# mackelab/poisson-gpfa

Hardware: AMD Instinct MI355X
Metric: EM iterations/sec (higher is better)
Workload: dtype f64

## Files before the change

### poisson-gpfa_amd/csrc/core.hip

```cpp
#include "ctx.h"
#include "model.h"
#include "dual.h"

using namespace pgpfa;

thread_local std::string g_err;
thread_local unsigned long long g_fail_count = 0;

int fail(const char* fmt, ...) {
  char buf[1024];
  va_list ap;
  va_start(ap, fmt);
  vsnprintf(buf, sizeof(buf), fmt, ap);
  va_end(ap);
  g_err = buf;
  ++g_fail_count;
  return 1;
}

int ensure_hbuf(pgpfa_ctx* c, size_t len) {
  if (len <= c->hbuf_len) return 0;
  if (c->hbuf) hipHostFree(c->hbuf);
  c->hbuf = nullptr;
  HIPC(hipHostMalloc((void**)&c->hbuf, len * sizeof(double)));
// ... 792 lines not shown
  rc |= dmalloc(c, &c->dual_tbl, (size_t)round_up(q, 128) * c->dual_ncol + 4096, true);
  rc |= dmalloc(c, &c->ppart, (size_t)p * (PACC_SPLITS + 1) * T * T + 256);
  c->vsmgp_ok.assign(R, 0);
  c->trial_snap.assign(R, -1);
  c->trial_dual.assign(R, 0);
  c->lam_resident.assign(R, 0);
  c->lam_valid.assign(R, 0);
  rc |= dmalloc(c, &c->Flr, slab * p + 256 * (size_t)c->Tp, true);
  rc |= dmalloc(c, &c->d_rank, p); rc |= dmalloc(c, &c->d_roff, p + 1); rc |= dmalloc(c, &c->d_roff16, p + 1);
  rc |= dmalloc(c, &c->d_cmap, (size_t)p * c->Tp + 2 * NB + 64); rc |= dmalloc(c, &c->d_nrtab, (size_t)p * c->Tp / 16 + 64);
  c->tab_cap = 4 * ((size_t)c->ld / 64 + 2 * (size_t)p + 4);
  rc |= dmalloc(c, &c->d_kr_ft, c->tab_cap); rc |= dmalloc(c, &c->d_kr_f, c->tab_cap);
  rc |= dmalloc(c, &c->sink, 128, true);
  rc |= dmalloc(c, &c->zero16, 2, true);
  rc |= dmalloc(c, &c->d_thin_ft, c->tab_cap); rc |= dmalloc(c, &c->d_thin_f, c->tab_cap); rc |= dmalloc(c, &c->d_thin_s, c->tab_cap);
  rc |= dmalloc(c, &c->Fbig, (size_t)c->ld * c->ld + 256 * (size_t)c->ld, true); rc |= dmalloc(c, &c->FTbig, (size_t)c->ld * c->ld + 256 * (size_t)c->ld, true);
  rc |= dmalloc(c, &c->Gbar, (size_t)T * p * p + 64); rc |= dmalloc(c, &c->Wtbar, (size_t)T * p * p + 64); rc |= dmalloc(c, &c->d_blk_lat, (size_t)p * c->Tp / 16 + 64); rc |= dmalloc(c, &c->d_blk_col, (size_t)p * c->Tp / 16 + 64);
  rc |= dmalloc(c, &c->vec, (size_t)q * (p + 1));
  rc |= dmalloc(c, &c->cdpart, (size_t)1024 * (p + 2) * q);
  rc |= dmalloc(c, &c->cdout, (size_t)(p + 2) * q + 8);
  rc |= dmalloc(c, &c->cdym, (size_t)(p + 1) * q + 8);
  rc |= dmalloc(c, &c->cdym_part, (size_t)1024 * (p + 1) * q);
  rc |= dmalloc(c, &c->last_trials, R);
  {
    const size_t NH = 1 + (size_t)(p + 1) + (size_t)(p + 1) * (p + 2) / 2;
    rc |= dmalloc(c, &c->cdhpart, (size_t)128 * NH * q);
    rc |= dmalloc(c, &c->cdhout, NH * q + 8);
    rc |= dmalloc(c, &c->cdcenter, (size_t)q * (p + 1));
    rc |= dmalloc(c, &c->cdpack, (size_t)q * (p + 3) + 8);
  }
  if (hipHostMalloc((void**)&c->h_pcg, 4 * sizeof(int), hipHostMallocMapped) != hipSuccess ||
      hipHostGetDevicePointer((void**)&c->d_hpcg, c->h_pcg, 0) != hipSuccess) { (void)hipGetLastError(); c->h_pcg = nullptr; c->d_hpcg = nullptr; }
  rc |= alloc_cholws(c, &c->kws, p * TAU_MULTI_MAX, c->Tp, true);
  c->kws.nact = round_up(T, 64);
  {
    const size_t nqmax = (size_t)p * TAU_MULTI_MAX;
    rc |= dmalloc(c, &c->tK, slab * nqmax); rc |= dmalloc(c, &c->tM, slab * nqmax); rc |= dmalloc(c, &c->tA1, slab * nqmax);
    rc |= dmalloc(c, &c->tA2, slab * nqmax);
    rc |= dmalloc(c, &c->tscal, 16 + 8 * nqmax); rc |= dmalloc(c, &c->tpart, 1024 + 64 * nqmax);
  }
  if (rc) { pgpfa_destroy(c); return 1; }
  e = hipStreamSynchronize(c->st);
  if (e != hipSuccess) { pgpfa_destroy(c); return fail("sync: %s", hipGetErrorString(e)); }
  if (const char* g = std::getenv("PGPFA_RANK_GRAN")) { const int v = std::atoi(g); if (v == 4 || v == 8 || v == 16) c->rank_gran = v; }
  c->info["n_pad"] = c->npad;
  c->info["counts_two_bytes"] = 0.0;
  c->info["trial_lengths_set"] = 0.0;
  c->info["observed_set"] = 0.0;
  c->info["last_cd_unobserved_neurons"] = 0.0;
  c->info["arena_bytes"] = 0.0;
  c->info["last_eps_wt_norm"] = 0.0;
  c->info["last_eps_wt_rms"] = 0.0;
  c->info["last_split_cov"] = 0.0;
  c->info["last_yt_mix_fused"] = 0.0;
  c->info["last_cov_f32"] = 0.0;
  c->info["last_cov_f32_fallbacks"] = 0.0;
  for (const char* k : {"plan_ms_total", "plans", "set_params_calls", "last_retry_ms", "last_dense_retries", "last_param_step", "last_param_step_prev",
                        "last_fallback_no_descent", "last_fallback_line_search", "last_fallback_outer_cap", "arena_grow_ms_total", "last_cold_restarts"}) c->info[k] = 0.0;
  *out = c;
  return 0;
}

int pgpfa_destroy(pgpfa_ctx* c) {
  if (!c) return 0;
  hipSetDevice(c->device);
  if (c->st) hipStreamSynchronize(c->st);
  if (c->comm) ncclCommDestroy(c->comm);
  for (void* p : c->allocs) hipFree(p);
  if (c->vsmgp) hipFree(c->vsmgp);
  if (c->Flr32) hipFree(c->Flr32);
  if (c->lam_keep) hipFree(c->lam_keep);
  if (c->split_buf) hipFree(c->split_buf);
  if (c->Yhi) hipFree(c->Yhi);
  if (c->trial_len) hipFree(c->trial_len);
  if (c->obs) hipFree(c->obs);
  arena_release(c);
  if (c->hbuf) hipHostFree(c->hbuf);
  if (c->dl_stage) hipHostFree(c->dl_stage);
  if (c->hibuf) hipHostFree(c->hibuf);
  if (c->ring) hipHostFree(c->ring);
  if (c->h_pcg) hipHostFree(c->h_pcg);
  if (c->h_seq) hipHostFree(c->h_seq);
  for (auto e : c->prof.pool) hipEventDestroy(e);
  if (c->st2) { hipStreamSynchronize(c->st2); hipStreamDestroy(c->st2); }
  if (c->tau_pin) hipHostFree(c->tau_pin);
  if (c->ev_tau_fork) hipEventDestroy(c->ev_tau_fork);
  if (c->ev_tau_done) hipEventDestroy(c->ev_tau_done);
  if (c->ev_fork) hipEventDestroy(c->ev_fork);
  if (c->ev_join) hipEventDestroy(c->ev_join);
  if (c->st) hipStreamDestroy(c->st);
  delete c;
  return 0;
}

int pgpfa_set_option(pgpfa_ctx* c, const char* key, double v) {
  if (!c || !key) return fail("null argument");
  const std::string k(key);
  if (k == "newton_xtol") c->xtol = v;
  else if (k == "newton_max_iter") c->max_iter = (int)v;
  else if (k == "use_mfma") {
    const bool was = c->mfma;
    c->mfma = (v != 0.0);
    if (c->have_params && c->rank_gran != 16 && was != c->mfma)
      CHK(pgpfa_set_params(c, std::vector<double>(c->hC).data(), std::vector<double>(c->hd).data(), std::vector<double>(c->htau).data()));
  }
  else if (k == "cd_mfma") c->cd_mfma = (v != 0.0);
  else if (k == "cd_hess_mfma") c->cd_hess_mfma = (v != 0.0);
  else if (k == "cross_kernel") c->cross_kernel = (v != 0.0);
  else if (k == "cd_debug") c->cd_debug = (int)v;
  else if (k == "pcg_fused") c->pcg_fused = (int)v;
  else if (k == "pcg_w32") c->pcg_w32 = (v != 0.0);
  else if (k == "pcg_form") c->pcg_form = (int)v;
  else if (k == "pcg_vec32") c->pcg_vec32 = (int)v;
  else if (k == "pcg_rx32") c->pcg_rx32 = (int)v;
  else if (k == "pcg_adapt") c->pcg_adapt = (int)v;
  else if (k == "pcg_xcd") c->pcg_xcd = (int)v;
  else if (k == "mt_fill") c->mt_fill = (int)v;
  else if (k == "overlap_factors") c->overlap_factors = (int)v;
  else if (k == "mix_slot") c->mix_slot = (int)v;
  else if (k == "yt_mix") c->yt_mix = (v != 0.0);
  else if (k == "pivchol_pairs") c->pivchol_pairs = (v != 0.0);
  else if (k == "vsm_b4") c->vsm_b4 = (int)v;
  else if (k == "poisson_tiles") c->poisson_tiles = (int)v;
  else if (k == "yt_mix_dbg") c->yt_mix_dbg = (int)v;
  else if (k == "yt_mix_dma") c->yt_mix_dma = (v != 0.0);
  else if (k == "syrk_dbg") c->syrk_dbg = (int)v;
  else if (k == "syrk_tile") c->syrk_tile = (int)v;
  else if (k == "mix_wide") c->mix_wide = (int)v;
  else if (k == "thin_products") {
    const bool was = c->thin_products >= 2;
    c->thin_products = (int)v;
    if (c->have_params && c->rank_gran != 16 && was != (c->thin_products >= 2))
      CHK(pgpfa_set_params(c, std::vector<double>(c->hC).data(), std::vector<double>(c->hd).data(), std::vector<double>(c->htau).data()));
  }
  else if (k == "copy_kernels") c->copy_kernels = (v != 0.0);
  else if (k == "chord") c->chord = (v != 0.0);
  else if (k == "shared_pcg") c->shared_pcg = (v != 0.0);
  else if (k == "time_newton") c->time_newton = (v != 0.0);
  else if (k == "pcg_trace") c->pcg_trace = (v != 0.0);
  else if (k == "measure_mix") { c->measure_mix = (v != 0.0); c->info["last_eps_wt_norm"] = 0.0; c->info["last_eps_wt_rms"] = 0.0; }
  else if (k == "pcg_retire") c->pcg_retire = (v != 0.0);
  else if (k == "split_cov") c->split_cov = (v != 0.0);
  else if (k == "split_max_norm") c->split_max_norm = v;
  else if (k == "cov_mode") c->cov_mode = (int)v;
  else if (k == "lowrank_tol") {
    const bool changed = c->lr_tol != v;
    c->lr_tol = v;
    if (c->have_params && changed)
      CHK(pgpfa_set_params(c, std::vector<double>(c->hC).data(), std::vector<double>(c->hd).data(), std::vector<double>(c->htau).data()));
  }
  else if (k == "keep_trial_vsmgp") c->keep_trial_vsmgp = (v != 0.0);
  else if (k == "dual_lowrank") c->dual_lowrank = (v != 0.0);
  else if (k == "dual_f32") c->dual_f32 = (int)v;
  else if (k == "laplace_f32") { if (v != 0.0 && v != 1.0 && v != 2.0) return fail("laplace_f32 is 0, 1 or 2"); c->laplace_f32 = (int)v; }
  else if (k == "laplace_evidence") { if (v != 0.0 && v != 1.0) return fail("laplace_evidence is 0 or 1"); c->laplace_evidence = (int)v; }
  else if (k == "sample_chunk_trials") { if (v < 0.0 || v != std::floor(v)) return fail("sample_chunk_trials is a count of trials, or 0"); c->sample_chunk = (int)v; }
  else if (k == "rates_chunk_trials") { if (v < 0.0 || v != std::floor(v)) return fail("rates_chunk_trials is a count of trials, or 0"); c->rates_chunk = (int)v; }
  else if (k == "slab_row_align") c->slab_row_align = (v != 0.0);
  else if (k == "vsm_mfma") c->vsm_mfma = (v != 0.0);
  else if (k == "dual_gemm") c->dual_gemm = (v != 0.0);
  else if (k == "extrapolate_start") c->extrapolate = (v != 0.0);
  else if (k == "extrapolate_beta") c->extrapolate_beta = v;
  else if (k == "extrapolate_guard") c->extrapolate_guard = v;
  else if (k == "start_guard") c->start_guard = (v != 0.0);
  else if (k == "shared_min") c->shared_min = (int)v;
  else if (k == "pcg_inner") c->pcg_inner_max = std::max(1, (int)v);
  else if (k == "pcg_eta0") c->pcg_eta0 = v;
  else if (k == "splitk_target") c->splitk_target = std::max(1, (int)v);
  else if (k == "small_tile_below") c->small_tile_below = (int)v;
  else if (k == "f32_tile64") c->f32_tile64 = (int)v;
  else if (k == "splitk_below64") c->splitk_below64 = (int)v;
  else if (k == "pcg_outer_max") c->pcg_outer_max = (int)v;
  else if (k == "chord_xtol") c->chord_xtol = v;
  else if (k == "chord_rho") c->chord_rho = v;
  else if (k == "chord_max_step") c->chord_max_step = v;
  else if (k == "chord_max") c->chord_max = (int)v;
  else if (k == "chunk_trials") { if (c->B > 0) return fail("chunk_trials must be set before the first E-step"); c->chunk_opt = (int)v; }
  else if (k == "workspace_headroom") c->arena_headroom = std::max(1.0, v);
  else if (k == "rank_gran") { if (v != 4.0 && v != 8.0 && v != 16.0) return fail("rank_gran is 4, 8 or 16"); c->rank_gran = (int)v; if (c->have_params) CHK(pgpfa_set_params(c, std::vector<double>(c->hC).data(), std::vector<double>(c->hd).data(), std::vector<double>(c->htau).data())); }
  else if (k == "workspace_pool") { if (c->arena_cap > 0) return fail("workspace_pool must be set before the first E-step"); c->use_pool = (v != 0.0); }
// ... 481 lines not shown
```

### poisson-gpfa_amd/csrc/cov.hip

```cpp
#include "ctx.h"
#include "model.h"
#include "split.h"
#include "ytmix.h"

using namespace pgpfa;

template <typename TIN>
void launch_post_vsm(pgpfa_ctx* c, const TIN* Mt, long long sM, int ncol, int ns, int full_range, const int* roff = nullptr, int ts = 0) {
  const int T = c->T, p = c->p;
  if (ts <= 0) ts = T;
  if (p > 10 && c->vsm_mfma) {
    const int CB = post_vsm_mfma_cb(p, sizeof(TIN) == 4);
    if (p <= 20 && c->vsm_b4) {
      constexpr int VW = 16 / (int)sizeof(TIN);
      const bool vec = c->vsm_b4 >= 2 && T % VW == 0 && ts % VW == 0 && c->ld % VW == 0 && sM % VW == 0 && (((size_t)Mt) & 15) == 0;
      auto go = [&](auto nbk, auto vv) {
        constexpr int NBK = decltype(nbk)::value;
        constexpr bool VEC = decltype(vv)::value;
        const size_t lds4 = (size_t)CB * post_vsm_b4_cs(p, VEC) * sizeof(TIN);
        constexpr int BINS = VEC ? 64 : 32;
        (void)hipFuncSetAttribute(reinterpret_cast<const void*>(&post_vsm_b4_kernel<NBK, TIN, VEC>), hipFuncAttributeMaxDynamicSharedMemorySize, (int)lds4);
        hipLaunchKernelGGL((post_vsm_b4_kernel<NBK, TIN, VEC>), dim3((T + BINS - 1) / BINS, ns), dim3(512), lds4, c->st, Mt, sM, c->ld, ncol, T, p, c->vsm,
                           c->ident, c->trial_of_slot, full_range, CB, roff, (int)GBN, ts);
      };
// ... 136 lines not shown
        a.ncmap = c->rank_compact ? round_up(c->rtot16, (int)NB) : 0;
        if (ytmix_lds(PW) + (size_t)a.ncmap * sizeof(int) > (size_t)160 * 1024) a.ncmap = 0;
        const size_t lds = ytmix_lds(PW) + (size_t)a.ncmap * sizeof(int);
        a.zero16 = c->zero16;
        const bool dma = c->yt_mix_dma && c->zero16 && (!a.cmap || a.ncmap > 0) && rpad % 2 == 0 && lw.sM % 2 == 0 && (reinterpret_cast<uintptr_t>(lw.Mt) & 15) == 0;
        auto launch = [&](auto kern) {
          (void)hipFuncSetAttribute(reinterpret_cast<const void*>(kern), hipFuncAttributeMaxDynamicSharedMemorySize, (int)lds);
          hipLaunchKernelGGL(kern, dim3((unsigned)(a.nbx * nb)), dim3(YTM_THREADS), lds, c->st, a);
        };
        if (dma) launch(&yt_mix_kernel<PW, true>); else launch(&yt_mix_kernel<PW, false>);
      }
    });
    prof_end(c);
  } else {
  prof_begin(c, TAG_MIX, (double)nb * T * (mix_cols * 8.0 + (double)p * ract * 4.0));
  if (p > 16)
    hipLaunchKernelGGL((mix_vsm_wide2_kernel<20, true>), dim3((T + 63) / 64, nb), dim3(256), 0, c->st, lw.H, (long long)lw.sH, c->ld, c->Gbin, sW, T, p, ract, c->eps,
                       c->vsm, c->ident, c->trial_of_slot, Ts, c->sink, D, sD, ldd);
  else
  dispatch_pw(p, [&](auto pw) {
    constexpr int PW = decltype(pw)::value;
    if constexpr (PW <= 10) {
      if (c->mix_slot >= 3 && p == PW && ract % 4 == 0) {
        (void)hipFuncSetAttribute(reinterpret_cast<const void*>(&mix_slot3_kernel<PW, 128, 2>), hipFuncAttributeMaxDynamicSharedMemorySize, (int)mix_slot_lds(PW, 128));
        hipLaunchKernelGGL((mix_slot3_kernel<PW, 128, 2>), dim3((T + 127) / 128, nb), dim3(256), mix_slot_lds(PW, 128), c->st, (const double*)lw.H, (long long)lw.sH, c->ld, D, sD, ldd,
                           c->Gbin, sW, T, ract, c->eps, c->vsm, c->ident, c->trial_of_slot, c->d_roff, ctile, Ts);
        return;
      }
      if (c->mix_slot >= 2 && p == PW && ract % 4 == 0) {
        (void)hipFuncSetAttribute(reinterpret_cast<const void*>(&mix_slot2_kernel<PW, 256, 2>), hipFuncAttributeMaxDynamicSharedMemorySize, (int)mix_slot_lds(PW, 256));
        hipLaunchKernelGGL((mix_slot2_kernel<PW, 256, 2>), dim3((T + 255) / 256, nb), dim3(256), mix_slot_lds(PW, 256), c->st, (const double*)lw.H, (long long)lw.sH, c->ld, D, sD, ldd,
                           c->Gbin, sW, T, ract, c->eps, c->vsm, c->ident, c->trial_of_slot, c->d_roff, ctile, Ts);
        return;
      }
      if (c->mix_slot) {
        (void)hipFuncSetAttribute(reinterpret_cast<const void*>(&mix_slot_kernel<PW, 256, 2>), hipFuncAttributeMaxDynamicSharedMemorySize, (int)mix_slot_lds(PW, 256));
        hipLaunchKernelGGL((mix_slot_kernel<PW, 256, 2>), dim3((T + 255) / 256, nb), dim3(256), mix_slot_lds(PW, 256), c->st, (const double*)lw.H, (long long)lw.sH, c->ld, D, sD, ldd,
                           c->Gbin, sW, T, p, ract, c->eps, c->vsm, c->ident, c->trial_of_slot, c->d_roff, ctile, Ts);
        return;
      }
    }
    if constexpr (PW <= 16)
      hipLaunchKernelGGL(mix_vsm_split_kernel<PW>, dim3((T + 63) / 64, nb), dim3(256), 0, c->st, (const double*)lw.H, (long long)lw.sH, c->ld, D, sD, ldd,
                         c->Gbin, sW, T, p, ract, c->eps, c->vsm, c->ident, c->trial_of_slot, c->d_roff, ctile, Ts);
  });
  prof_end(c);
  }
  const int sps = std::max(1, (nb + PACC_SPLITS - 1) / PACC_SPLITS);
  const int ngroups = (nb + sps - 1) / sps;
  {
    SyrkF16Args a{};
    a.D = D; a.sD = sD; a.ldd = ldd; a.ts = Ts; a.part = c->ppart;
    a.T = T; a.p = p; a.ract = ract; a.nslots = nb; a.sps = sps; a.ngroups = ngroups;
    a.dbg = c->syrk_dbg;
    const int t256 = (T + 255) / 256;
    const bool big = c->syrk_tile >= 256 && T > 256 && (Ts & 3) == 0 && (ldd & 3) == 0 && t256 * 256 <= Ts && (((size_t)D) & 15) == 0 && (sD & 3) == 0;
    a.tiles = big ? t256 : (T + 127) / 128; a.ntiles = a.tiles * (a.tiles + 1) / 2;
    const long long blocks = (long long)a.ntiles * ngroups * p;
    prof_begin(c, TAG_VSM, 3.0 * (double)nb * ract * T * T * p);
    if (big) {
      const size_t lds = (size_t)4 * 2 * 256 * 32 * sizeof(_Float16);
      (void)hipFuncSetAttribute(reinterpret_cast<const void*>(&syrk256_f16x2_kernel), hipFuncAttributeMaxDynamicSharedMemorySize, (int)lds);
      hipLaunchKernelGGL(syrk256_f16x2_kernel, dim3((unsigned)blocks), dim3(512), lds, c->st, a);
    } else {
      hipLaunchKernelGGL(syrk_f16x2_kernel, dim3((unsigned)blocks), dim3(256), 0, c->st, a);
    }
    prof_end(c);
  }
  const int spsS = std::max(1, (nb + NS - 1) / NS);
  for (int k = 0; k < p; ++k) {
    const int rk = c->rk[k], r0 = c->roff[k] & ~15;
    const int rrow = c->roff[k];
    const int kw = ract - r0;
    if (kw <= 0 || rk <= 0) {
      HIPC(hipMemsetAsync(T1 + (size_t)k * tt, 0, tt * sizeof(double), c->st));
      HIPC(hipMemsetAsync(Xfull + (size_t)k * tt, 0, tt * sizeof(double), c->st));
      continue;
    }
    const double* A0 = lw.Mt + rrow + (size_t)r0 * rpad;
    auto seg = [&](int sper, bool is_x, double* out) -> int {
      const int nfull = nb / sper, rem = nb - nfull * sper;
      for (int part = 0; part < 2; ++part) {
        const int first = part ? nfull * sper : 0, per = part ? rem : sper, ng = part ? (rem ? 1 : 0) : nfull;
        if (ng == 0 || per == 0) continue;
        GemmP g{};
        g.A = A0 + (size_t)first * lw.sM; g.sA = (long long)per * lw.sM; g.lda = rpad;
        g.kseg = kw; g.sAseg = lw.sM;
        g.K = per * kw; g.alpha = 1.0; g.beta = 0.0; g.slots = nullptr; g.nbatch = ng; g.kflags = 0; g.bm = 64;
        g.M = rk;
        if (is_x) {
          g.B = reinterpret_cast<const double*>(D + (size_t)first * sD + (size_t)k * Ts + (size_t)r0 * ldd);
          g.sB = (long long)per * sD; g.ldb = ldd; g.sBseg = sD; g.b_f32 = 1;
          g.N = T; g.mode = GEMM_FULL;
          g.C = out + (size_t)(part ? nfull : 0) * rk * T; g.sC = (long long)rk * T; g.ldc = rk;
        } else {
          g.B = g.A; g.sB = g.sA; g.ldb = rpad; g.sBseg = lw.sM;
          g.N = rk; g.mode = GEMM_LOWER;
          g.C = out + (size_t)(part ? nfull : 0) * rk * rk; g.sC = (long long)rk * rk; g.ldc = rk;
        }
        CHK(gemm(c, false, g));
      }
      return 0;
    };
    CHK(seg(spsS, false, Spart));
    if (c->cross_kernel && c->mfma && rk % 16 == 0 && kw % 16 == 0) {
      for (int row0 = 0; row0 < rk; row0 += 128) {
        CrossArgs ca{};
        ca.A = A0; ca.sM = lw.sM; ca.lda = rpad;
        ca.D = D + (size_t)k * Ts + (size_t)r0 * ldd; ca.sD = sD; ca.ldd = ldd;
        ca.C = Xpart; ca.sC = (long long)rk * T;
        ca.rk = std::min(128, rk - row0); ca.T = T; ca.kw = kw; ca.nslots = nb; ca.sps = sps;
// ... 484 lines not shown
```

### poisson-gpfa_amd/csrc/ctx.h

```cpp
#pragma once
#include <hip/hip_runtime.h>
#include <rccl/rccl.h>

#include <algorithm>
#include <limits>
#include <chrono>
#include <cmath>
#include <cstdarg>
#include <cstdio>
#include <cstring>
#include <deque>
#include <functional>
#include <map>
#include <string>
#include <type_traits>
#include <vector>

#include <mutex>
#include <rocprofiler-sdk-roctx/roctx.h>
#include "../../include/pgpfa.h"
#include "types.h"

using namespace pgpfa;

// ... 144 lines not shown
  bool live_gemm_collect = false;
  std::vector<std::pair<std::string, double>> live_gemms;
  bool pcg_retire = true;
  int* h_pcg = nullptr; int* d_hpcg = nullptr;
  float* W32 = nullptr;
  double* sc_part2 = nullptr;
  int pcg_fused = 1; bool pcg_w32 = true;
  int mt_fill = 1;
  int pcg_xcd = 1;
  int pcg_adapt = 1;
  int pcg_form = 2;
  int pcg_rx32 = 1;
  int pcg_vec32 = 1;
  double *Sv = nullptr, *cg_scal = nullptr;
  double *GbT = nullptr, *WbT = nullptr;
  double *sc_rz = nullptr, *sc_pq = nullptr, *sc_rr = nullptr, *sc_rr0 = nullptr, *sc_pack = nullptr;
  double* Flr = nullptr;
  double* Gbin = nullptr;
  int *d_rank = nullptr, *d_blk_lat = nullptr, *d_blk_col = nullptr, *d_roff = nullptr;
  int *d_kr_ft = nullptr, *d_kr_f = nullptr;
  int kr_ft_len = 0, kr_f_len = 0;
  int ntab_ft = 0, ntab_f = 0; size_t tab_cap = 0;
  int *d_thin_ft = nullptr, *d_thin_f = nullptr, *d_thin_s = nullptr;
  int nthin_ft = 0, nthin_f = 0, nthin_s = 0;
  int thin_products = 2;
  double *Fbig = nullptr, *FTbig = nullptr, *Gbar = nullptr, *Wtbar = nullptr;
  std::vector<int> rk, roff;
  std::vector<int> rr, roff16;
  int rtot = 0, rpad = 0, rtot16 = 0;
  int rank_gran = 4;
  bool rank_compact = false;
  int *d_roff16 = nullptr, *d_cmap = nullptr, *d_nrtab = nullptr;
  int cov_mode = 0;
  double lr_tol = 1e-10;
  bool plan_lowrank = false;
  size_t slab_elems = 0, mt_elems = 0, ws_mark = 0;
  char* arena = nullptr; size_t arena_cap = 0, arena_off = 0; int arena_mode = 0;
  int vmm = 0; size_t va_size = 0, vmm_gran = 0, vmm_granule = (size_t)1 << 30;
  std::vector<std::pair<hipMemGenericAllocationHandle_t, size_t>> vmm_chunks;
  double arena_headroom = 2.0;
  bool mt_dirty = false;
  bool last_cov_lowrank = false;
  bool shared_pcg = true;
  bool pcg_trace = false;
  double* zero16 = nullptr;
  double* sink = nullptr;
  int mix_wide = 1;
  int poisson_tiles = 2;
  int vsm_b4 = 2;
  int pivchol_pairs = 1;
  int yt_mix = 1;
  int syrk_tile = 256;
  int syrk_dbg = 0;
  int yt_mix_dma = 1;
  int yt_mix_dbg = 0;
  int mix_slot = 3;
  bool cross_kernel = true;
  bool measure_mix = false;
  bool time_newton = false;
  int shared_min = 16, pcg_inner_min = 2, pcg_inner_max = 16, pcg_outer_max = 12;
  double pcg_eta0 = 1e-2;
  int splitk_target = 1280;
  int f32_tile64 = 1;
  int small_tile_below = 1 << 30;
  int splitk_below64 = 400;
  double *sc_f = nullptr, *sc_qxx = nullptr, *sc_qdx = nullptr, *sc_qdd = nullptr, *sc_dec = nullptr, *sc_smax = nullptr, *sc_alpha = nullptr;
  int *trial_of_slot = nullptr, *list_a = nullptr, *list_b = nullptr, *ident = nullptr;
  int* mask_of_slot = nullptr;
  bool mask_active = false;
  CholWS kws{};
  double *tK = nullptr, *tM = nullptr, *tA1 = nullptr, *tA2 = nullptr, *tscal = nullptr, *tpart = nullptr;
  double* hbuf = nullptr; size_t hbuf_len = 0;
  struct DlEntry { void* host; size_t off, bytes; };
  PcgCtl fused_ctl_host{};
  char* dl_stage = nullptr; size_t dl_used = 0; std::vector<DlEntry> dl_pending;
  char* dl_stage_dev = nullptr; char* ring_dev = nullptr;
  unsigned* h_seq = nullptr; unsigned* d_seq = nullptr; unsigned seq_next = 0;
  bool copy_kernels = true;
  unsigned long long dl_fail_mark = 0;
  int* hibuf = nullptr; size_t hibuf_len = 0;
  char* ring = nullptr; size_t ring_slot = 0; int ring_cur = 0, ring_pending = 0;
  std::map<std::string, double> info;
  std::vector<void*> allocs;
  size_t bytes = 0;
  Prof prof;
  ncclComm_t comm = nullptr;
  int rank = 0, nranks = 1;
  double* commbuf = nullptr; size_t commbuf_len = 0;
  double* rates_tbl = nullptr; double rates_tbl_params = -1.0;
  int rates_chunk = 0;
  int sample_chunk = 0;
};

template <typename T>
int dmalloc(pgpfa_ctx* c, T** out, size_t count, bool zero = false) {
  void* p = nullptr;
  const size_t bytes = std::max<size_t>(count, 1) * sizeof(T);
  if (c->arena_mode) {
    const size_t aligned = (bytes + 255) & ~(size_t)255;
    *out = nullptr;
    if (c->arena_mode == 2) {
      if (c->arena_off + aligned > c->arena_cap) return fail("workspace arena overflow (%zu + %zu > %zu bytes)", c->arena_off, aligned, c->arena_cap);
      p = c->arena + c->arena_off;
      if (zero && hipMemsetAsync(p, 0, bytes, c->st) != hipSuccess) return fail("hipMemset failed");
      *out = reinterpret_cast<T*>(p);
    }
// ... 135 lines not shown
```

### poisson-gpfa_amd/csrc/split.h

```cpp
#pragma once
#include <type_traits>
#include <hip/hip_runtime.h>

namespace pgpfa {

typedef _Float16 half8_t __attribute__((ext_vector_type(8)));
typedef float float4v_t __attribute__((ext_vector_type(4)));

constexpr float SPLIT_SCALE = 2048.0f;


template <int PW>
__global__ __launch_bounds__(256, 2) void mix_vsm_split_kernel(const double* __restrict__ Yt, long long sY, int ldy, float* __restrict__ D, long long sD,
                                                            int ldd, const double* __restrict__ G, long long sG, int T, int p, int rpad, double eps,
                                                            double* __restrict__ vsm, const int* __restrict__ slots,
                                                            const int* __restrict__ trial_of_slot, const int* __restrict__ roff, int col_tile, int ts) {
  constexpr int PP = PW * PW, LD = PP + 1, NPAIR = PW * (PW + 1) / 2;
  __shared__ double Gs[64 * LD];
  const int pp = p * p;
  const int slot = slots[blockIdx.y];
  const int t0 = blockIdx.x * 64;
  const int nt = min(64, T - t0);
  const double* gbase = G + (size_t)slot * sG + (size_t)t0 * pp;
  if (p < PW)
// ... 317 lines not shown
          m[u][a] += gg * v[u][c2];
          if (c2 != a) m[u][c2] += gg * v[u][a];
        }
      }
#pragma unroll
    for (int u = 0; u < U; ++u)
#pragma unroll
      for (int k = 0; k < PW; ++k) rsrc_store_f32(d, voff * 4u, (unsigned)((b0 + u) * ldd + k * ts) * 4u, (float)(v[u][k] - m[u][k]));
    asm volatile("" ::: "memory");
    if (bnext < ract) fetch(bnext, v);
#pragma unroll
    for (int u = 0; u < U; ++u)
#pragma unroll
      for (int a = 0; a < PW; ++a)
#pragma unroll
        for (int c2 = 0; c2 <= a; ++c2) acc[a * (a + 1) / 2 + c2] += m[u][a] * m[u][c2];
  };
  double vA[U][PW], vB[U][PW];
  const int first = half * U;
  if (first < ract) fetch(first, vA);
  if (first + 2 * U < ract) fetch(first + 2 * U, vB);
  for (int b0 = first; b0 < ract; b0 += 4 * U) {
    trip(b0, vA, b0 + 4 * U);
    if (b0 + 2 * U < ract) trip(b0 + 2 * U, vB, b0 + 6 * U);
  }
  __syncthreads();
  if (half == 0) {
#pragma unroll
    for (int i = 0; i < NPAIR; ++i) acc[i] += eps * gs[i * NB];
  }
  __syncthreads();
  if (half == 1) {
#pragma unroll
    for (int i = 0; i < NPAIR; ++i) gs[i * NB] = acc[i];
  }
  __syncthreads();
  if (half != 0 || t >= T) return;
  double* vdst = vsm + ((size_t)trial_of_slot[slot] * T + t) * pp;
#pragma unroll
  for (int a = 0; a < PW; ++a)
#pragma unroll
    for (int c2 = 0; c2 <= a; ++c2) {
      const double val = acc[a * (a + 1) / 2 + c2] + gs[(a * (a + 1) / 2 + c2) * NB];
      vdst[a * p + c2] = val;
      vdst[c2 * p + a] = val;
    }
}

struct SyrkF16Args {
  const float* D; long long sD; int ldd, ts;
  double* part;
  int T, p, ract, nslots, sps, ngroups, tiles, ntiles;
  int dbg;
};

inline __global__ __launch_bounds__(256, 2) void syrk_f16x2_kernel(SyrkF16Args a) {
  constexpr int BT = 128, KS = 32, LS = 32;
  auto lidx = [](int row, int chunk) { return row * LS + ((chunk ^ ((4 - ((row >> 2) & 3)) & 3)) << 3); };
  __shared__ __attribute__((aligned(16))) _Float16 Ah[2][BT * LS], Al[2][BT * LS], Bh[2][BT * LS], Bl[2][BT * LS];
  const int tid = threadIdx.x;
  const int lane = tid & 63;
  const int wave = __builtin_amdgcn_readfirstlane(tid >> 6);
  const int wm = wave >> 1, wn = wave & 1;
  const int nbatch = a.ngroups * a.p;
  int b, tile;
  {
    const int bid = blockIdx.x;
    const int full = nbatch >> 3, per_group = a.ntiles << 3, grp = bid / per_group;
    if (grp < full) { const int r = bid - grp * per_group; tile = r >> 3; b = (grp << 3) + (r & 7); }
    else { const int m = nbatch - (full << 3); const int r = bid - full * per_group; tile = r / m; b = (full << 3) + (r - tile * m); }
  }
  int tj = 0, rem = tile;
  while (rem >= a.tiles - tj) { rem -= a.tiles - tj; ++tj; }
  const int ti = tj + rem;
  const int k = b / a.ngroups, g = b - k * a.ngroups;
  const int i0 = ti * BT, j0 = tj * BT;
  const bool diag = (ti == tj);
  const int s_begin = g * a.sps, s_end = min(a.nslots, s_begin + a.sps);
  const bool wave_live = (i0 + wm * 64 < a.T) && (j0 + wn * 64 < a.T) && !(i0 + wm * 64 + 63 < j0 + wn * 64);

  float4v_t acc[4][4];
#pragma unroll
  for (int mi = 0; mi < 4; ++mi)
#pragma unroll
    for (int ni = 0; ni < 4; ++ni) acc[mi][ni] = float4v_t{0.f, 0.f, 0.f, 0.f};

  const bool is_b = tid >= 128;
  const int rq = tid & 31, co = (tid >> 5) & 3;
  const int row0 = (is_b ? j0 : i0) + 4 * rq;
  const bool stage = !(is_b && diag);
  const bool vec = ((a.ts & 3) == 0) && ((a.ldd & 3) == 0) && (i0 + BT <= a.ts) && (j0 + BT <= a.ts) && ((((size_t)a.D) & 15) == 0) && ((a.sD & 3) == 0);
  float4v_t vA[8], vB[8];
  const int steps_per_slot = (a.ract + KS - 1) / KS;
  const int nsteps = (s_end - s_begin) * steps_per_slot;
  auto load = [&](auto vecc, int step, float4v_t (&v4)[8]) {
    constexpr bool VEC = decltype(vecc)::value;
    const int st = min(step, nsteps - 1);
    const int s = s_begin + st / steps_per_slot;
    const int c0 = (st % steps_per_slot) * KS + co * 8;
    const float* base = stage ? a.D + (size_t)s * a.sD + (size_t)k * a.ts : a.D;
#pragma unroll
    for (int j = 0; j < 8; ++j) {
      const int c = c0 + j;
      const bool in = stage && c < a.ract;
      const size_t off = (size_t)(in ? c : 0) * a.ldd;
      float4v_t x;
// ... 53 lines not shown
      al[mi] = *reinterpret_cast<const half8_t*>(&Al[buf][r]);
    }
#pragma unroll
    for (int ni = 0; ni < 4; ++ni) {
      const int r = lidx(wn * 64 + ni * 16 + l15, l4);
      bh[ni] = *reinterpret_cast<const half8_t*>(&Bhs[r]);
      bl[ni] = *reinterpret_cast<const half8_t*>(&Bls[r]);
    }
#pragma unroll
    for (int mi = 0; mi < 4; ++mi)
#pragma unroll
      for (int ni = 0; ni < 4; ++ni) {
        acc[mi][ni] = __builtin_amdgcn_mfma_f32_16x16x32_f16(bh[ni], ah[mi], acc[mi][ni], 0, 0, 0);
        acc[mi][ni] = __builtin_amdgcn_mfma_f32_16x16x32_f16(bh[ni], al[mi], acc[mi][ni], 0, 0, 0);
        acc[mi][ni] = __builtin_amdgcn_mfma_f32_16x16x32_f16(bl[ni], ah[mi], acc[mi][ni], 0, 0, 0);
      }
  };
  auto run = [&](auto vecc) {
    if (nsteps <= 0) return;
    constexpr bool FAST = decltype(vecc)::value;
    auto ld = [&](int step, float4v_t (&v4)[8]) { if constexpr (FAST) load_fast(v4); else load(vecc, step, v4); };
    ld(0, vA);
    ld(1, vB);
    store(0, vA);
    if (!(a.dbg & 8)) __syncthreads();
    for (int step = 0; step < nsteps; step += 2) {
      ld(step + 2, vA);
      multiply(0);
      if (step + 1 < nsteps) store(1, vB);
      if (!(a.dbg & 8)) __syncthreads();
      if (step + 1 >= nsteps) break;
      ld(step + 3, vB);
      multiply(1);
      if (step + 2 < nsteps) store(0, vA);
      if (!(a.dbg & 8)) __syncthreads();
    }
  };
  if (vec) run(std::true_type{}); else run(std::false_type{});
  if (!wave_live) return;
  double* C = a.part + (size_t)(k * a.ngroups + g) * a.T * a.T;
  const double inv = 1.0 / ((double)SPLIT_SCALE * (double)SPLIT_SCALE);
#pragma unroll
  for (int mi = 0; mi < 4; ++mi) {
    const int i = i0 + wm * 64 + mi * 16 + l15;
    if (i >= a.T) continue;
#pragma unroll
    for (int ni = 0; ni < 4; ++ni)
#pragma unroll
      for (int r = 0; r < 4; ++r) {
        const int j = j0 + wn * 64 + ni * 16 + 4 * l4 + r;
        if (j >= a.T) continue;
        C[(size_t)j * a.T + i] = (double)acc[mi][ni][r] * inv;
      }
  }
}

inline __global__ __launch_bounds__(512, 1) void syrk256_f16x2_kernel(SyrkF16Args a) {
  constexpr int BT = 256, KS = 32, LS = 32;
  auto lidx = [](int row, int chunk) { return row * LS + ((chunk ^ ((4 - ((row >> 2) & 3)) & 3)) << 3); };
  extern __shared__ __attribute__((aligned(16))) _Float16 syrk256_lds[];
  _Float16* Ah = syrk256_lds;
  _Float16* Al = Ah + 2 * BT * LS;
  _Float16* Bh = Al + 2 * BT * LS;
  _Float16* Bl = Bh + 2 * BT * LS;
  const int tid = threadIdx.x;
  const int lane = tid & 63;
  const int wave = __builtin_amdgcn_readfirstlane(tid >> 6);
  const int wm = wave >> 1, wn = wave & 1;
  const int nbatch = a.ngroups * a.p;
  int b, tile;
  {
    const int bid = blockIdx.x;
    const int full = nbatch >> 3, per_group = a.ntiles << 3, grp = bid / per_group;
    if (grp < full) { const int r = bid - grp * per_group; tile = r >> 3; b = (grp << 3) + (r & 7); }
    else { const int m = nbatch - (full << 3); const int r = bid - full * per_group; tile = r / m; b = (full << 3) + (r - tile * m); }
  }
  int tj = 0, rem = tile;
  while (rem >= a.tiles - tj) { rem -= a.tiles - tj; ++tj; }
  const int ti = tj + rem;
  const int k = b / a.ngroups, g = b - k * a.ngroups;
  const int i0 = ti * BT, j0 = tj * BT;
  const bool diag = (ti == tj);
  const int s_begin = g * a.sps, s_end = min(a.nslots, s_begin + a.sps);
  const bool wave_live = (i0 + wm * 64 < a.T) && (j0 + wn * 128 < a.T) && !(i0 + wm * 64 + 63 < j0 + wn * 128);

  float4v_t acc[4][8];
#pragma unroll
  for (int mi = 0; mi < 4; ++mi)
#pragma unroll
    for (int ni = 0; ni < 8; ++ni) acc[mi][ni] = float4v_t{0.f, 0.f, 0.f, 0.f};

  const bool is_b = tid >= 256;
  const int rq = tid & 63, co = (tid >> 6) & 3;
  const int row0 = (is_b ? j0 : i0) + 4 * rq;
  const bool stage = !(is_b && diag);
  const int steps_per_slot = (a.ract + KS - 1) / KS;
  const int nsteps = (s_end - s_begin) * steps_per_slot;
  int cur_s = s_begin, cur_c = 0;
  const unsigned voff = (unsigned)(stage ? (co * 8) * a.ldd + row0 : 0) * 4u;
  float4v_t v[8];
  auto load_fast = [&]() {
    typedef unsigned u32x4 __attribute__((ext_vector_type(4)));
    const __amdgpu_buffer_rsrc_t rs = wave_uniform_rsrc(a.D + (size_t)cur_s * a.sD, (size_t)a.ract * a.ldd * sizeof(float));
    const unsigned soff = (unsigned)(k * a.ts + cur_c * KS * a.ldd) * 4u;
#pragma unroll
    for (int j = 0; j < 8; ++j) {
      const u32x4 w = __builtin_amdgcn_raw_buffer_load_b128(rs, (int)voff, (int)(soff + (unsigned)(j * a.ldd) * 4u), 0);
      v[j] = float4v_t{__uint_as_float(w.x), __uint_as_float(w.y), __uint_as_float(w.z), __uint_as_float(w.w)};
    }
    if (cur_c + 1 < steps_per_slot) ++cur_c;
    else if (cur_s + 1 < s_end) { ++cur_s; cur_c = 0; }
  };
  auto store = [&](int buf) {
    if (!stage) return;
    _Float16* Hh = (is_b ? Bh : Ah) + buf * BT * LS;
    _Float16* Hl = (is_b ? Bl : Al) + buf * BT * LS;
#pragma unroll
    for (int r = 0; r < 4; ++r) {
      half8_t h, l;
#pragma unroll
      for (int j = 0; j < 8; ++j) {
        const float x = v[j][r] * SPLIT_SCALE;
        const _Float16 hx = (_Float16)x;
        h[j] = hx;
        l[j] = (_Float16)(x - (float)hx);
      }
      *reinterpret_cast<half8_t*>(&Hh[lidx(4 * rq + r, co)]) = h;
      *reinterpret_cast<half8_t*>(&Hl[lidx(4 * rq + r, co)]) = l;
    }
  };
  const int l15 = lane & 15, l4 = lane >> 4;
  auto multiply = [&](int buf) {
    if (!wave_live) return;
    const _Float16* As_h = Ah + buf * BT * LS;
    const _Float16* As_l = Al + buf * BT * LS;
    const _Float16* Bs_h = (diag ? Ah : Bh) + buf * BT * LS;
    const _Float16* Bs_l = (diag ? Al : Bl) + buf * BT * LS;
    half8_t ah[4], al[4];
#pragma unroll
    for (int mi = 0; mi < 4; ++mi) {
      const int r = lidx(wm * 64 + mi * 16 + l15, l4);
      ah[mi] = *reinterpret_cast<const half8_t*>(&As_h[r]);
      al[mi] = *reinterpret_cast<const half8_t*>(&As_l[r]);
    }
#pragma unroll
    for (int half = 0; half < 2; ++half) {
      half8_t bh[4], bl[4];
#pragma unroll
      for (int ni = 0; ni < 4; ++ni) {
        const int r = lidx(wn * 128 + half * 64 + ni * 16 + l15, l4);
        bh[ni] = *reinterpret_cast<const half8_t*>(&Bs_h[r]);
        bl[ni] = *reinterpret_cast<const half8_t*>(&Bs_l[r]);
      }
#pragma unroll
      for (int mi = 0; mi < 4; ++mi)
#pragma unroll
        for (int ni = 0; ni < 4; ++ni) {
          float4v_t c = acc[mi][half * 4 + ni];
          c = __builtin_amdgcn_mfma_f32_16x16x32_f16(bh[ni], ah[mi], c, 0, 0, 0);
          c = __builtin_amdgcn_mfma_f32_16x16x32_f16(bh[ni], al[mi], c, 0, 0, 0);
          c = __builtin_amdgcn_mfma_f32_16x16x32_f16(bl[ni], ah[mi], c, 0, 0, 0);
          acc[mi][half * 4 + ni] = c;
        }
    }
  };
  if (nsteps > 0) {
    load_fast();
    store(0);
    __syncthreads();
    for (int step = 0; step < nsteps; ++step) {
      if (step + 1 < nsteps) load_fast();
      multiply(step & 1);
      if (step + 1 < nsteps) store((step + 1) & 1);
      __syncthreads();
    }
  }
  if (!wave_live) return;
  double* C = a.part + (size_t)(k * a.ngroups + g) * a.T * a.T;
  const double inv = 1.0 / ((double)SPLIT_SCALE * (double)SPLIT_SCALE);
#pragma unroll
  for (int mi = 0; mi < 4; ++mi) {
    const int i = i0 + wm * 64 + mi * 16 + l15;
    if (i >= a.T) continue;
#pragma unroll
    for (int ni = 0; ni < 8; ++ni)
#pragma unroll
      for (int r = 0; r < 4; ++r) {
        const int j = j0 + wn * 128 + ni * 16 + 4 * l4 + r;
        if (j >= a.T) continue;
        C[(size_t)j * a.T + i] = (double)acc[mi][ni][r] * inv;
      }
  }
}

struct CrossArgs {
  const double* A; long long sM; int lda;
  const void* D; long long sD; int ldd;
  double* C; long long sC;
  int rk, T, kw, nslots, sps;
  int row0, ldc;
};

template <int NTR, typename TB, bool LOWER>
__global__ __launch_bounds__(256) void cross_term_kernel(CrossArgs a) {
  constexpr int GK = 16;
  constexpr int RS = NTR * 16 + ((NTR & 1) ? 0 : 16);
  constexpr int NA = (GK * NTR * 16 + 255) / 256;
  __shared__ double As[2][GK][RS];
  __shared__ double Bs[2][GK][64 + 16];
  const int tid = threadIdx.x;
  const int lane = tid & 63, wave = __builtin_amdgcn_readfirstlane(tid >> 6);
  const int l15 = lane & 15, l4 = lane >> 4;
  const int t0 = blockIdx.x * 64;
  const int g = blockIdx.y;
  const int s_begin = g * a.sps, s_end = min(a.nslots, s_begin + a.sps);
  const int cps = a.kw / GK;
  const int nchunks = (s_end - s_begin) * cps;
  const int rk = a.rk;
  const TB* Dall = reinterpret_cast<const TB*>(a.D);
  const int ct = blockIdx.x * 4 + wave;
  const bool wave_live = t0 + wave * 16 < a.T;

  double raA[NA], raB[NA];
  TB rbA[4], rbB[4];
  int cur_s = s_begin, cur_c = 0;
  size_t aoff[NA], doff[4];
#pragma unroll
// ... 178 lines not shown
```

Measured before the change: 12.40.

## Add balanced diagonal-tile path to 256-wide split-f16 SYRK kernel

Diagonal 256x256 tiles of the SYRK kernel now take a dedicated path. It splits the lower triangle into 36 32x32 units, spread by a compile-time table over 8 waves with at most 5 units each and equal load per SIMD. In the old path a diagonal tile left whole waves idle on its upper half while the rest did 64x128 blocks. The new path only stages the A operand, so it also halves staging work and LDS traffic on diagonal tiles. It adds register pressure from 5 accumulator sets, plus debug flags that can skip conversion, products or barriers.

```diff
diff --git a/poisson-gpfa_amd/csrc/core.hip b/poisson-gpfa_amd/csrc/core.hip
--- a/poisson-gpfa_amd/csrc/core.hip
+++ b/poisson-gpfa_amd/csrc/core.hip
@@ -868,6 +868,7 @@
   c->info["last_eps_wt_norm"] = 0.0;
   c->info["last_eps_wt_rms"] = 0.0;
   c->info["last_split_cov"] = 0.0;
+  c->info["last_syrk_tile"] = 0.0;
   c->info["last_yt_mix_fused"] = 0.0;
   c->info["last_cov_f32"] = 0.0;
   c->info["last_cov_f32_fallbacks"] = 0.0;
@@ -942,6 +943,7 @@
   else if (k == "yt_mix_dma") c->yt_mix_dma = (v != 0.0);
   else if (k == "syrk_dbg") c->syrk_dbg = (int)v;
   else if (k == "syrk_tile") c->syrk_tile = (int)v;
+  else if (k == "syrk_diag") c->syrk_diag = (int)v;
   else if (k == "mix_wide") c->mix_wide = (int)v;
   else if (k == "thin_products") {
     const bool was = c->thin_products >= 2;
diff --git a/poisson-gpfa_amd/csrc/cov.hip b/poisson-gpfa_amd/csrc/cov.hip
--- a/poisson-gpfa_amd/csrc/cov.hip
+++ b/poisson-gpfa_amd/csrc/cov.hip
@@ -212,11 +212,12 @@
     SyrkF16Args a{};
     a.D = D; a.sD = sD; a.ldd = ldd; a.ts = Ts; a.part = c->ppart;
     a.T = T; a.p = p; a.ract = ract; a.nslots = nb; a.sps = sps; a.ngroups = ngroups;
-    a.dbg = c->syrk_dbg;
+    a.dbg = c->syrk_dbg; a.diag = c->syrk_diag ? 1 : 0;
     const int t256 = (T + 255) / 256;
     const bool big = c->syrk_tile >= 256 && T > 256 && (Ts & 3) == 0 && (ldd & 3) == 0 && t256 * 256 <= Ts && (((size_t)D) & 15) == 0 && (sD & 3) == 0;
     a.tiles = big ? t256 : (T + 127) / 128; a.ntiles = a.tiles * (a.tiles + 1) / 2;
     const long long blocks = (long long)a.ntiles * ngroups * p;
+    c->info["last_syrk_tile"] = big ? 256.0 : 128.0;
     prof_begin(c, TAG_VSM, 3.0 * (double)nb * ract * T * T * p);
     if (big) {
       const size_t lds = (size_t)4 * 2 * 256 * 32 * sizeof(_Float16);
diff --git a/poisson-gpfa_amd/csrc/ctx.h b/poisson-gpfa_amd/csrc/ctx.h
--- a/poisson-gpfa_amd/csrc/ctx.h
+++ b/poisson-gpfa_amd/csrc/ctx.h
@@ -220,6 +220,7 @@
   int yt_mix = 1;
   int syrk_tile = 256;
   int syrk_dbg = 0;
+  int syrk_diag = 1;
   int yt_mix_dma = 1;
   int yt_mix_dbg = 0;
   int mix_slot = 3;
diff --git a/poisson-gpfa_amd/csrc/split.h b/poisson-gpfa_amd/csrc/split.h
--- a/poisson-gpfa_amd/csrc/split.h
+++ b/poisson-gpfa_amd/csrc/split.h
@@ -393,6 +393,7 @@
   double* part;
   int T, p, ract, nslots, sps, ngroups, tiles, ntiles;
   int dbg;
+  int diag;
 };
 
 inline __global__ __launch_bounds__(256, 2) void syrk_f16x2_kernel(SyrkF16Args a) {
@@ -552,6 +553,190 @@
         if (j >= a.T) continue;
         C[(size_t)j * a.T + i] = (double)acc[mi][ni][r] * inv;
       }
+  }
+}
+
+struct SyrkDiagUnits {
+  int n[8];
+  int row[8][5], col[8][5];
+};
+constexpr SyrkDiagUnits syrk_diag_units() {
+  SyrkDiagUnits t{};
+  for (int m = 0; m < 4; ++m) {
+    int& na = t.n[m];
+    int& nb = t.n[m + 4];
+    for (int c = 0; c < 5; ++c) { t.row[m][na] = 7 - m; t.col[m][na] = c; ++na; }
+    for (int c = 5; c <= 7 - m; ++c) { t.row[m + 4][nb] = 7 - m; t.col[m + 4][nb] = c; ++nb; }
+    for (int c = 0; c <= m; ++c) { t.row[m + 4][nb] = m; t.col[m + 4][nb] = c; ++nb; }
+  }
+  return t;
+}
+constexpr bool syrk_diag_units_ok(const SyrkDiagUnits& t) {
+  int seen[8][8] = {};
+  int simd[4] = {};
+  for (int w = 0; w < 8; ++w) {
+    if (t.n[w] < 0 || t.n[w] > 5) return false;
+    simd[w & 3] += t.n[w];
+    for (int s = 0; s < t.n[w]; ++s) {
+      if (t.row[w][s] < 0 || t.row[w][s] > 7 || t.col[w][s] < 0 || t.col[w][s] > t.row[w][s]) return false;
+      ++seen[t.row[w][s]][t.col[w][s]];
+    }
+  }
+  for (int r = 0; r < 8; ++r)
+    for (int c = 0; c <= r; ++c)
+      if (seen[r][c] != 1) return false;
+  return simd[0] == simd[1] && simd[1] == simd[2] && simd[2] == simd[3];
+}
+static_assert(syrk_diag_units_ok(syrk_diag_units()), "syrk256 diagonal tiles: the unit table must cover the lower 32 x 32 units once, <= 5 per wave, evenly over the SIMDs");
+constexpr unsigned long long syrk_diag_word(int w) {
+  const SyrkDiagUnits t = syrk_diag_units();
+  unsigned long long x = 0;
+  for (int s = 0; s < t.n[w]; ++s) {
+    const bool first = s == 0 || t.row[w][s] != t.row[w][s - 1];
+    x |= (unsigned long long)(t.row[w][s] | (t.col[w][s] << 3) | 64 | (first ? 128 : 0)) << (8 * s);
+  }
+  return x;
+}
+
+__device__ __forceinline__ void syrk256_diag_tile(const SyrkF16Args& a, _Float16* Ah, _Float16* Al, int k, int g, int i0, int s_begin, int s_end) {
+  constexpr int BT = 256, KS = 32, LS = 32;
+  typedef _Float16 half4_t __attribute__((ext_vector_type(4)));
+  auto lidx = [](int row, int chunk) { return row * LS + ((chunk ^ ((4 - ((row >> 2) & 3)) & 3)) << 3); };
+  const int tid = threadIdx.x;
+  const int lane = tid & 63;
+  const int wave = __builtin_amdgcn_readfirstlane(tid >> 6);
+  static constexpr unsigned long long words[8] = {syrk_diag_word(0), syrk_diag_word(1), syrk_diag_word(2), syrk_diag_word(3),
+                                                  syrk_diag_word(4), syrk_diag_word(5), syrk_diag_word(6), syrk_diag_word(7)};
+  const unsigned long long word = words[wave];
+  int ur[5], uc[5];
+  bool live[5], first[5];
+#pragma unroll
+  for (int s = 0; s < 5; ++s) {
+    const unsigned e = (unsigned)(word >> (8 * s)) & 0xffu;
+    ur[s] = e & 7; uc[s] = (e >> 3) & 7;
+    live[s] = (e & 64) && (i0 + 32 * ur[s] < a.T) && (i0 + 32 * uc[s] < a.T);
+    first[s] = (e & 128) != 0;
+  }
+  float4v_t acc[5][2][2];
+#pragma unroll
+  for (int s = 0; s < 5; ++s)
+#pragma unroll
+    for (int mi = 0; mi < 2; ++mi)
+#pragma unroll
+      for (int ni = 0; ni < 2; ++ni) acc[s][mi][ni] = float4v_t{0.f, 0.f, 0.f, 0.f};
+
+  const int rq = tid & 63, c4 = wave;
+  const int steps_per_slot = (a.ract + KS - 1) / KS;
+  const int nsteps = (s_end - s_begin) * steps_per_slot;
+  int cur_s = s_begin, cur_c = 0;
+  const unsigned voff = (unsigned)((c4 * 4) * a.ldd + i0 + 4 * rq) * 4u;
+  float4v_t v[4];
+  auto load_fast = [&]() {
+    typedef unsigned u32x4 __attribute__((ext_vector_type(4)));
+    const __amdgpu_buffer_rsrc_t rs = wave_uniform_rsrc(a.D + (size_t)cur_s * a.sD, (size_t)a.ract * a.ldd * sizeof(float));
+    const unsigned soff = (unsigned)(k * a.ts + cur_c * KS * a.ldd) * 4u;
+#pragma unroll
+    for (int j = 0; j < 4; ++j) {
+      const u32x4 w = __builtin_amdgcn_raw_buffer_load_b128(rs, (int)voff, (int)(soff + (unsigned)(j * a.ldd) * 4u), 0);
+      v[j] = float4v_t{__uint_as_float(w.x), __uint_as_float(w.y), __uint_as_float(w.z), __uint_as_float(w.w)};
+    }
+    if (cur_c + 1 < steps_per_slot) ++cur_c;
+    else if (cur_s + 1 < s_end) { ++cur_s; cur_c = 0; }
+  };
+  const bool noconv = (a.dbg & 1) != 0;
+  auto store = [&](int buf) {
+    _Float16* Hh = Ah + buf * BT * LS;
+    _Float16* Hl = Al + buf * BT * LS;
+    if (noconv) {
+#pragma unroll
+      for (int r = 0; r < 4; ++r) {
+        const int at = lidx(4 * rq + r, c4 >> 1) + 4 * (c4 & 1);
+        *reinterpret_cast<half4_t*>(&Hh[at]) = half4_t{0, 0, 0, 0};
+        *reinterpret_cast<half4_t*>(&Hl[at]) = half4_t{0, 0, 0, 0};
+      }
+      return;
+    }
+#pragma unroll
+    for (int r = 0; r < 4; ++r) {
+      half4_t h, l;
+#pragma unroll
+      for (int j = 0; j < 4; ++j) {
+        const float x = v[j][r] * SPLIT_SCALE;
+        const _Float16 hx = (_Float16)x;
+        h[j] = hx;
+        l[j] = (_Float16)(x - (float)hx);
+      }
+      const int at = lidx(4 * rq + r, c4 >> 1) + 4 * (c4 & 1);
+      *reinterpret_cast<half4_t*>(&Hh[at]) = h;
+      *reinterpret_cast<half4_t*>(&Hl[at]) = l;
+    }
+  };
+  const int l15 = lane & 15, l4 = lane >> 4;
+  const int lfrag = lidx(l15, l4);
+  const bool noprod = (a.dbg & 2) != 0;
+  auto multiply = [&](int buf) {
+    if (noprod) return;
+    const _Float16* As_h = Ah + buf * BT * LS + lfrag;
+    const _Float16* As_l = Al + buf * BT * LS + lfrag;
+    half8_t ah[2] = {}, al[2] = {};
+#pragma unroll
+    for (int s = 0; s < 5; ++s) {
+      if (!live[s]) continue;
+      if (first[s]) {
+#pragma unroll
+        for (int mi = 0; mi < 2; ++mi) {
+          ah[mi] = *reinterpret_cast<const half8_t*>(&As_h[(32 * ur[s] + 16 * mi) * LS]);
+          al[mi] = *reinterpret_cast<const half8_t*>(&As_l[(32 * ur[s] + 16 * mi) * LS]);
+        }
+      }
+      half8_t bh[2], bl[2];
+#pragma unroll
+      for (int ni = 0; ni < 2; ++ni) {
+        bh[ni] = *reinterpret_cast<const half8_t*>(&As_h[(32 * uc[s] + 16 * ni) * LS]);
+        bl[ni] = *reinterpret_cast<const half8_t*>(&As_l[(32 * uc[s] + 16 * ni) * LS]);
+      }
+#pragma unroll
+      for (int mi = 0; mi < 2; ++mi)
+#pragma unroll
+        for (int ni = 0; ni < 2; ++ni) {
+          float4v_t c = acc[s][mi][ni];
+          c = __builtin_amdgcn_mfma_f32_16x16x32_f16(bh[ni], ah[mi], c, 0, 0, 0);
+          c = __builtin_amdgcn_mfma_f32_16x16x32_f16(bh[ni], al[mi], c, 0, 0, 0);
+          c = __builtin_amdgcn_mfma_f32_16x16x32_f16(bl[ni], ah[mi], c, 0, 0, 0);
+          acc[s][mi][ni] = c;
+        }
+    }
+  };
+  const bool nobar = (a.dbg & 8) != 0;
+  if (nsteps > 0) {
+    load_fast();
+    store(0);
+    if (!nobar) __syncthreads();
+    for (int step = 0; step < nsteps; ++step) {
+      if (step + 1 < nsteps) load_fast();
+      multiply(step & 1);
+      if (step + 1 < nsteps) store((step + 1) & 1);
+      if (!nobar) __syncthreads();
+    }
+  }
+  double* C = a.part + (size_t)(k * a.ngroups + g) * a.T * a.T;
+  const double inv = 1.0 / ((double)SPLIT_SCALE * (double)SPLIT_SCALE);
+#pragma unroll
+  for (int s = 0; s < 5; ++s) {
+    if (!live[s]) continue;
+#pragma unroll
+    for (int mi = 0; mi < 2; ++mi) {
+      const int i = i0 + 32 * ur[s] + 16 * mi + l15;
+      if (i >= a.T) continue;
+#pragma unroll
+      for (int ni = 0; ni < 2; ++ni)
+#pragma unroll
+        for (int r = 0; r < 4; ++r) {
+          const int j = i0 + 32 * uc[s] + 16 * ni + 4 * l4 + r;
+          if (j >= a.T) continue;
+          C[(size_t)j * a.T + i] = (double)acc[s][mi][ni][r] * inv;
+        }
+    }
   }
 }
 
@@ -582,6 +767,10 @@
   const int i0 = ti * BT, j0 = tj * BT;
   const bool diag = (ti == tj);
   const int s_begin = g * a.sps, s_end = min(a.nslots, s_begin + a.sps);
+  if (diag && a.diag) {
+    syrk256_diag_tile(a, Ah, Al, k, g, i0, s_begin, s_end);
+    return;
+  }
   const bool wave_live = (i0 + wm * 64 < a.T) && (j0 + wn * 128 < a.T) && !(i0 + wm * 64 + 63 < j0 + wn * 128);
 
   float4v_t acc[4][8];
@@ -611,10 +800,19 @@
     if (cur_c + 1 < steps_per_slot) ++cur_c;
     else if (cur_s + 1 < s_end) { ++cur_s; cur_c = 0; }
   };
+  const bool noconv = (a.dbg & 1) != 0, noprod = (a.dbg & 2) != 0, nobar = (a.dbg & 8) != 0;
   auto store = [&](int buf) {
     if (!stage) return;
     _Float16* Hh = (is_b ? Bh : Ah) + buf * BT * LS;
     _Float16* Hl = (is_b ? Bl : Al) + buf * BT * LS;
+    if (noconv) {
+#pragma unroll
+      for (int r = 0; r < 4; ++r) {
+        *reinterpret_cast<half8_t*>(&Hh[lidx(4 * rq + r, co)]) = half8_t{0, 0, 0, 0, 0, 0, 0, 0};
+        *reinterpret_cast<half8_t*>(&Hl[lidx(4 * rq + r, co)]) = half8_t{0, 0, 0, 0, 0, 0, 0, 0};
+      }
+      return;
+    }
 #pragma unroll
     for (int r = 0; r < 4; ++r) {
       half8_t h, l;
@@ -631,7 +829,7 @@
   };
   const int l15 = lane & 15, l4 = lane >> 4;
   auto multiply = [&](int buf) {
-    if (!wave_live) return;
+    if (!wave_live || noprod) return;
     const _Float16* As_h = Ah + buf * BT * LS;
     const _Float16* As_l = Al + buf * BT * LS;
     const _Float16* Bs_h = (diag ? Ah : Bh) + buf * BT * LS;
@@ -667,12 +865,12 @@
   if (nsteps > 0) {
     load_fast();
     store(0);
-    __syncthreads();
+    if (!nobar) __syncthreads();
     for (int step = 0; step < nsteps; ++step) {
       if (step + 1 < nsteps) load_fast();
       multiply(step & 1);
       if (step + 1 < nsteps) store((step + 1) & 1);
-      __syncthreads();
+      if (!nobar) __syncthreads();
     }
   }
   if (!wave_live) return;
```

Result: no change. 12.47 (median of 3 runs) (+0.6%).
